# llGuy/madrona_renderer

Hardware: AMD Instinct MI355X
Metric: rendered views/sec (whole node), N worlds x 64x64 RGB+depth (higher is better)
Workload: dtype f32

## Files before the change

include/mrx.h:

```cpp
#ifndef MRX_H
#define MRX_H

#include <stddef.h>
#include <stdint.h>

#ifdef __cplusplus
extern "C" {
#endif

#define MRX_ABI_VERSION 4

enum {
    MRX_OK = 0,
    MRX_E_INVALID = -1,
    MRX_E_NO_DEVICE = -2,
    MRX_E_HIP = -3,
    MRX_E_ASSET = -4,
    MRX_E_UNSUPPORTED = -5
};

enum { MRX_MODE_RASTERIZER = 0, MRX_MODE_RAYTRACER = 1 };

typedef struct {
    float position[3];
// ... 220 lines not shown
                  uint32_t pass_rows, float *out_flow);

int mrx_copy_to_host(mrx_renderer *r, int which, void *dst, uint64_t bytes);

int mrx_refresh_objects(mrx_renderer *r);

int mrx_num_shards(mrx_renderer *r);
mrx_renderer *mrx_shard(mrx_renderer *r, int shard);
void *mrx_buffer_shard(mrx_renderer *r, int shard, int which, int64_t dims[4], int *ndim,
                       int *dtype, int *device);
int64_t mrx_shard_first_world(mrx_renderer *r, int shard);
int64_t mrx_shard_split(uint32_t num_worlds, uint32_t shard, uint32_t num_shards);

enum {
    MRX_ENTRY_NONE = 0, MRX_ENTRY_GROUP_FAST = 1, MRX_ENTRY_GROUP = 2, MRX_ENTRY_CHUNKED = 3,
    MRX_ENTRY_BRUTE = 4, MRX_ENTRY_BVH = 5
};
int mrx_raster_entry(mrx_renderer *r);
enum {
    MRX_FORM_UNIFORM = 0, MRX_FORM_PV = 1, MRX_FORM_PVL = 2, MRX_FORM_C = 3, MRX_FORM_PVLC = 4, MRX_FORM_M = 5,
    MRX_FORM_PVLM = 6, MRX_FORM_N = 7, MRX_FORM_NPV = 8, MRX_FORM_L = 9, MRX_FORM_LN = 10, MRX_FORM_PVM = 11
};
typedef struct {
    int32_t form;
    int32_t slots;
} mrx_kernel_form_t;
int mrx_kernel_form(mrx_renderer *r, mrx_kernel_form_t *out);
enum { MRX_BVH_KERNEL_NONE = 0, MRX_BVH_KERNEL_TILE = 1, MRX_BVH_KERNEL_FLAT = 2 };
typedef struct {
    int32_t kernel;
    uint32_t tile_w, tile_h;
// ... 33 lines not shown
int mrx_obj_objects(const char *path, uint32_t *first_tri, uint32_t capacity);
int mrx_decode_png(const char *path, uint8_t **rgba, uint32_t *width,
                   uint32_t *height);
int mrx_decode_texture(const char *path, uint8_t **rgba, uint32_t *width,
                       uint32_t *height);
int mrx_decode_bc7(const uint8_t *blocks, uint32_t num_blocks, uint8_t *rgba );
int64_t mrx_describe_obj_materials(const char *path, char *json, uint64_t capacity);
int mrx_blas_check(const float *tri_pos , uint32_t num_tris, uint32_t *num_nodes,
                   uint32_t *depth, uint32_t *num_leaves);
void mrx_free(void *p);
uint32_t mrx_dispatch_min_tris(uint32_t base, uint32_t num_views, int textured, uint32_t width, uint32_t height,
                               uint32_t num_cus);
uint32_t mrx_group_fill(uint32_t num_cus);
int mrx_dispatch_flat(int raytracer, uint32_t num_views, uint32_t width, uint32_t height, uint32_t max_world_triangles,
                      uint32_t max_world_instances, uint32_t num_cus);

int mrx_set_view_projection(mrx_renderer *r, uint32_t first_view, uint32_t count, const mrx_projection *proj);
int mrx_view_projection(mrx_renderer *r, uint32_t first_view, uint32_t count, mrx_projection *out);
int mrx_projection_constants(uint32_t width, uint32_t height, int render_mode, mrx_projection proj, float out[6]);

int mrx_set_world_light(mrx_renderer *r, uint32_t first_world, uint32_t count, const mrx_light *lights);
int mrx_world_light(mrx_renderer *r, uint32_t first_world, uint32_t count, mrx_light *out);
int mrx_light_constants(mrx_light light, float out[5]);

int mrx_set_instance_materials(mrx_renderer *r, uint32_t first_row, uint32_t count, const int32_t *materials);
int mrx_instance_materials(mrx_renderer *r, uint32_t first_row, uint32_t count, int32_t *out);

int mrx_set_instance_labels(mrx_renderer *r, uint32_t first_row, uint32_t count, const int32_t *labels);
int mrx_instance_labels(mrx_renderer *r, uint32_t first_row, uint32_t count, int32_t *out);

// ... 9 lines not shown
```

madrona_renderer_amd/build.py:

```python
import os
import shutil
import subprocess
import sys
import sysconfig

HERE = os.path.dirname(os.path.abspath(__file__))
ROOT = os.path.dirname(HERE)
CSRC = os.path.join(HERE, "csrc")
ARCH = "gfx950"

HIP_SOURCES = ["raster.hip", "bvh.hip", "resolve.hip", "unproject.hip", "boxes.hip", "observe.hip", "rays.hip", "rays_host.cpp", "flow.hip", "flow_host.cpp", "bvh.cpp", "mrx_api.cpp", "scene.cpp", "stages.cpp", "shards.cpp", "host_tools.cpp", "assets.cpp", "ktx2.cpp"]
HIP_DEPS = HIP_SOURCES + ["raster.hpp", "raster_dev.hpp", "bvh.hpp", "resolve.hpp", "unproject.hpp", "boxes.hpp", "observe.hpp", "rays.hpp", "rays_core.hpp", "flow.hpp", "flow_core.hpp", "assets.hpp", "bc7_tables.inc",
                          "renderer.hpp", "shards.hpp", "error.hpp",
                          "../../include/mrx.h"]
MGR_SOURCES = ["manager.cpp"]
MGR_DEPS = MGR_SOURCES + ["../../include/madrona_mi355/manager.hpp",
                          "../../include/madrona_mi355/types.hpp", "../../include/mrx.h"]
PY_SOURCES = ["py_module.cpp", "manager.cpp"]


def ext_suffix():
    return sysconfig.get_config_var("EXT_SUFFIX") or ".so"


def lib_path():
    return os.path.join(HERE, "libmrx_hip.so")

# ... 188 lines not shown
```

madrona_renderer_amd/csrc/host_tools.cpp:

```cpp
#include "renderer.hpp"

#include "assets.hpp"
#include "boxes.hpp"
#include "rays.hpp"

extern "C" {

int mrx_projection_constants(uint32_t width, uint32_t height, int render_mode, mrx_projection proj, float out[6])
{
    if (!out)
        return fail(MRX_E_INVALID, "null output");
    if (render_mode != MRX_MODE_RASTERIZER && render_mode != MRX_MODE_RAYTRACER)
        return fail(MRX_E_INVALID, "bad render_mode");
    const bool rt = render_mode == MRX_MODE_RAYTRACER;
    mrx::ViewProj c;
    const int rc = projectionConstants(width, rt ? width : height, rt, proj, c);
    if (rc != MRX_OK)
        return rc;
    out[0] = c.sx; out[1] = c.ox; out[2] = c.sz; out[3] = c.oz; out[4] = c.invNear; out[5] = c.s6bPad;
    return MRX_OK;
}

int mrx_light_constants(mrx_light light, float out[5])
{
// ... 178 lines not shown
}

uint32_t mrx_dispatch_min_tris(uint32_t base, uint32_t num_views, int textured, uint32_t width, uint32_t height,
                               uint32_t num_cus)
{
    return mrx::bvhDispatchMinTris(base ? base : mrx::kBvhMinTris, num_views, textured != 0, width, height, num_cus);
}

uint32_t mrx_group_fill(uint32_t num_cus) { return mrx::groupFill(num_cus); }

int mrx_dispatch_flat(int raytracer, uint32_t num_views, uint32_t width, uint32_t height, uint32_t max_world_triangles,
                      uint32_t max_world_instances, uint32_t num_cus)
{
    return mrx::bvhDispatchFlat(raytracer != 0, num_views, width, raytracer ? width : height, max_world_triangles,
                                max_world_instances, num_cus) ? 1 : 0;
}

int mrx_blas_check(const float *tri_pos, uint32_t num_tris, uint32_t *num_nodes, uint32_t *depth,
                   uint32_t *num_leaves)
{
    if ((!tri_pos && num_tris) || !num_nodes || !depth || !num_leaves)
        return fail(MRX_E_INVALID, "null argument");
    using namespace mrx;
    std::vector<ObjTri> tris(num_tris);
    for (uint32_t t = 0; t < num_tris; ++t)
        std::memcpy(tris[t].p, tri_pos + 9 * (size_t)t, 36);
    BlasSet b;
    buildBlas(tris.data(), { 0 }, { (int32_t)num_tris }, b);
    *num_nodes = (uint32_t)b.nodes.size();
    *depth = b.maxDepth;
// ... 66 lines not shown
```

madrona_renderer_amd/csrc/manager.cpp:

```cpp
#include "../../include/madrona_mi355/manager.hpp"
#include "../../include/mrx.h"

#include <algorithm>
#include <cstdio>
#include <cstdlib>
#include <stdexcept>
#include <string>
#include <vector>

namespace madRender {

namespace detail {
static bool g_throwOnError = false;
void setThrowOnError(bool v) { g_throwOnError = v; }

[[noreturn]] static void fatal(const char *msg)
{
    if (g_throwOnError)
        throw std::runtime_error(msg);
    std::fprintf(stderr, "FATAL: %s\n", msg);
    std::fflush(stderr);
    std::abort();
}
[[noreturn]] static void fatal(const std::string &msg) { fatal(msg.c_str()); }
// ... 302 lines not shown
    return accepted(mrx_set_instance_labels(impl_->r, first, count, labels));
}

void Manager::instanceLabels(uint32_t first, uint32_t count, int32_t *out) const
{
    check(mrx_instance_labels(impl_->r, first, count, out));
}

int Manager::placement(float *candUs, int capacity, float *keptUs) const
{
    return mrx_placement(impl_->r, candUs, capacity, keptUs);
}

const char *Manager::rasterEntry() const
{
    static const char *const names[] = {"none", "group-fast", "group", "chunked", "brute", "bvh"};
    const int e = mrx_raster_entry(impl_->r);
    if (e < 0 || e >= (int)(sizeof names / sizeof names[0]))
        detail::fatal(mrx_last_error());
    return names[e];
}

Manager::KernelFormInfo Manager::kernelForm() const
{
    static const char *const names[] = {"Uniform", "PV", "PVL", "C", "PVLC", "M", "PVLM", "N", "NPV", "L", "LN", "PVM"};
    mrx_kernel_form_t f {};
    check(mrx_kernel_form(impl_->r, &f));
    if (f.form < 0 || f.form >= (int)(sizeof names / sizeof names[0]))
        detail::fatal("mrx_kernel_form: unknown form");
    return KernelFormInfo { names[f.form], f.slots };
}
// ... 13 lines not shown
```

madrona_renderer_amd/csrc/mrx_api.cpp:

```cpp
#include "renderer.hpp"

#include <chrono>
#include <utility>

#include "boxes.hpp"
#include "observe.hpp"

constexpr size_t kOutPeriod = 512u << 10;
static size_t outPhase(const char *env, size_t dflt)
{
    if (const char *dbg = std::getenv(env))
        return (size_t)std::atoll(dbg) << 10;
    return dflt;
}
bool firstKindIsOneBlock(size_t px)
{
    if (const char *dbg = std::getenv("MRX_OUT_KIND"))
        return dbg[0] == 'o';
    return px * 4 < (128ull << 20);
}

hipError_t allocOutputs(size_t px, bool wantRgb, bool wantDepth, bool wantIds, bool oneAllocation,
                        DevBuf<uint32_t> &rgb, DevBuf<float> &depth, DevBuf<int32_t> &ids,
                        bool wantNormal, DevBuf<uint32_t> &normal)
// ... 775 lines not shown
        if (const int src = settle(r))
            return src;
    if (!r)
        return fail(MRX_E_INVALID, "null renderer");
    if (!r->shards.empty())
        return shardsRun(r, kCmdSync);
    MRX_HIP(hipSetDevice(r->device));
    MRX_HIP(hipStreamSynchronize(r->stream));
    return MRX_OK;
}

void *mrx_stream(mrx_renderer *r) { return r ? (void *)r->stream : nullptr; }

static_assert(mrx::kEntryNone == MRX_ENTRY_NONE && mrx::kEntryGroupFast == MRX_ENTRY_GROUP_FAST &&
                  mrx::kEntryGroup == MRX_ENTRY_GROUP && mrx::kEntryChunked == MRX_ENTRY_CHUNKED &&
                  mrx::kEntryBrute == MRX_ENTRY_BRUTE && mrx::kEntryBvh == MRX_ENTRY_BVH,
              "raster.hpp RasterEntry and mrx.h MRX_ENTRY_* disagree");

int mrx_raster_entry(mrx_renderer *r)
{
    if (!r)
        return fail(MRX_E_INVALID, "null renderer");
    return r->shards.empty() ? r->lastEntry : r->shards[0]->lastEntry;
}

#define MRX_FORM_SAME(name, NAME) ((int)mrx::KernelForm::name == MRX_FORM_##NAME)
static_assert(MRX_FORM_SAME(Uniform, UNIFORM) && MRX_FORM_SAME(PV, PV) && MRX_FORM_SAME(PVL, PVL) && MRX_FORM_SAME(C, C) &&
                  MRX_FORM_SAME(PVLC, PVLC) && MRX_FORM_SAME(M, M) && MRX_FORM_SAME(PVLM, PVLM) && MRX_FORM_SAME(N, N) &&
                  MRX_FORM_SAME(NPV, NPV) && MRX_FORM_SAME(L, L) && MRX_FORM_SAME(LN, LN) && MRX_FORM_SAME(PVM, PVM),
              "raster.hpp KernelForm and mrx.h MRX_FORM_* disagree");
#undef MRX_FORM_SAME
// ... 473 lines not shown
```

madrona_renderer_amd/csrc/raster.hip:

```cpp
#include <hip/hip_runtime.h>
#include <algorithm>
#include <cstdlib>

#include "raster.hpp"
#include "raster_dev.hpp"

namespace mrx {
namespace {

constexpr int kWavesPerBlock = 4;
constexpr int kBruteThreads = kWave * kWavesPerBlock;
constexpr int kChunkedThreads = kWave * kWavesPerBlock, kChunkedWavesPerSimd = 3;
constexpr int kChunk = 64;
constexpr int kHot = 16;
constexpr int kBandRows = 16;
constexpr int kBlocksPerBand = 16;

struct WaveLds {
    float hot[kChunk][kHot];
    float cold[kChunk][kCold];
};

struct TileCtx {
    uint32_t view, tileX0, tileY0;
    uint32_t triBegin, numTris;
    int lx, ly;
};

// ... 244 lines not shown
void rasterBruteKernel(const RasterParams p)
{
    bruteKernelBody<IDS, MULTI, OUT, false>(p);
}

template <KernelForm F, bool IDS, bool MULTI>
__global__ __launch_bounds__(kBruteThreads)
void rasterBruteFormKernel(const RasterParams p)
{
    static_assert(F == KernelForm::PV || F == KernelForm::N || F == KernelForm::NPV, "the forms of this family");
    bruteKernelBody<IDS, MULTI, kOutByPointer, formFlags(F).pv, formFlags(F).nrm>(p);
}

constexpr uint32_t kNearFree = 1u << 16;

template <int S0, int S1>
__device__ __forceinline__ uint32_t classifyStrips(const TriPlanes &c, uint32_t tileX0,
                                                   uint32_t tileY0, float invNear, float invFar,
                                                   bool &nearOk)
{
    const float X0 = (float)tileX0, Y0 = (float)tileY0;
    const float xa0 = c.A0 < 0.0f ? X0 : X0 + 31.0f;
    const float xa1 = c.A1 < 0.0f ? X0 : X0 + 31.0f;
    const float xa2 = c.A2 < 0.0f ? X0 : X0 + 31.0f;
    const float xdh = c.Dx < 0.0f ? X0 : X0 + 31.0f;
    const float xdl = c.Dx < 0.0f ? X0 + 31.0f : X0;
    const float yb0 = c.B0 < 0.0f ? Y0 : Y0 + 7.0f;
    const float yb1 = c.B1 < 0.0f ? Y0 : Y0 + 7.0f;
    const float yb2 = c.B2 < 0.0f ? Y0 : Y0 + 7.0f;
    const float ydh = c.Dy < 0.0f ? Y0 : Y0 + 7.0f;
    const float ydl = c.Dy < 0.0f ? Y0 + 7.0f : Y0;
    uint32_t mask = 0;
    float dmax = -__builtin_inff();
#pragma unroll
    for (int s = S0; s < S1; ++s) {
        const float dy = (float)(8 * s);
        const float r0 = __builtin_fmaf(c.B0, yb0 + dy, c.C0);
        const float r1 = __builtin_fmaf(c.B1, yb1 + dy, c.C1);
        const float r2 = __builtin_fmaf(c.B2, yb2 + dy, c.C2);
        const float rh = __builtin_fmaf(c.Dy, ydh + dy, c.Dc);
        const float rl = __builtin_fmaf(c.Dy, ydl + dy, c.Dc);
        const bool yin = (Y0 + dy + 7.0f >= c.bbY0) && (Y0 + dy <= c.bbY1);
#pragma unroll
        for (int hf = 0; hf < 2; ++hf) {
            const float dx = (float)(32 * hf);
            const float e0 = __builtin_fmaf(c.A0, xa0 + dx, r0);
            const float e1 = __builtin_fmaf(c.A1, xa1 + dx, r1);
            const float e2 = __builtin_fmaf(c.A2, xa2 + dx, r2);
            const float dh = __builtin_fmaf(c.Dx, xdh + dx, rh);
            const float dl = __builtin_fmaf(c.Dx, xdl + dx, rl);
            const bool xin = (X0 + dx + 31.0f >= c.bbX0) && (X0 + dx <= c.bbX1);
            const bool possible = (fminf(fminf(e0, e1), e2) >= 0.0f) &&
                                  (dh > invFar) && (dl <= invNear) && xin && yin;
            mask |= possible ? (1u << (2 * s + hf)) : 0u;
            dmax = fmaxf(dmax, dh);
        }
    }
    nearOk = dmax <= invNear;
    return mask;
}

__device__ __forceinline__ uint32_t classifyRegions(const TriPlanes &c, const TileCtx &t,
                                                    float invNear, float invFar)
{
    bool nearOk;
    uint32_t mask = classifyStrips<0, 8>(c, t.tileX0, t.tileY0, invNear, invFar, nearOk);
    if (nearOk)
        mask |= kNearFree;
    return mask;
}


template <bool NEAR>
__device__ __forceinline__ void pixelTest(const PlanePairs &q, f32x2 r01, f32x2 r2d, float px,
                                          float invNear, int32_t kv, float &best, int32_t &bid)
{
    const f32x2 pp = { px, px };
    const f32x2 e01 = fma2(q.A01, pp, r01);
    const f32x2 e2d = fma2(q.A2D, pp, r2d);
    bool in = (fminf(fminf(e01.x, e01.y), e2d.x) >= 0.0f) & (e2d.y > best);
    if (NEAR)
        in = in & (e2d.y <= invNear);
    best = in ? e2d.y : best;
    bid = in ? kv : bid;
}

template <bool NEAR, int IDSHIFT>
__device__ __forceinline__ void rasterRegion(const float (*planes)[16], uint64_t act, int recBase,
                                             const float (&px)[kRegionBlocks], float py,
                                             float invNear,
                                             float (&best)[kRegionBlocks],
                                             int32_t (&bid)[kRegionBlocks])
{
    const f32x2 yy = { py, py };
    for (; act != 0; act &= act - 1) {
        const int k = recBase + __builtin_ctzll(act);
        const PlanePairs q = loadPlanes(planes, k);
        const f32x2 r01 = fma2(q.B01, yy, q.C01);
        const f32x2 r2d = fma2(q.B2D, yy, q.C2D);
#pragma unroll
        for (int b = 0; b < kRegionBlocks; ++b)
            pixelTest<NEAR>(q, r01, r2d, px[b], invNear, k << IDSHIFT, best[b], bid[b]);
    }
}

template <bool IDS, bool NRM = false>
__device__ __forceinline__ void outputRegion(const RasterParams &p, const TileCtx &t,
                                             uint32_t fx0, uint32_t fy, float invFar,
                                             const float (&best)[kRegionBlocks],
                                             const uint32_t (&rgba)[kRegionBlocks],
                                             const int32_t (&id)[kRegionBlocks],
                                             const uint32_t *nrm = nullptr)
{
    float dep[kRegionBlocks];
#pragma unroll
    for (int b = 0; b < kRegionBlocks; ++b)
        dep[b] = best[b] > invFar ? __builtin_amdgcn_rcpf(best[b]) : 0.0f;
    if (fy >= p.nslow || (p.debugSkip & 1u))
        return;
// ... 175 lines not shown
    static constexpr int kRecs = SLOTS <= kChunk ? kChunk + 16 : SLOTS;
    static constexpr int kBackground = kRecs;
    float planes[kRecs][16];
    uint32_t live[kRecs];
    float shade[kRecs + 1][4];
    float cold[kRecs][kCold];
    uint32_t masks[groupTilesMax(SLOTS) * (SLOTS <= kChunk ? kChunk : SLOTS)];
    uint32_t tileInfo[kGroupTilesMax][4];
    float tileNear[PV ? kGroupTilesMax : 1];
    uint32_t nextItem;
    uint8_t itemOrder[kGroupTilesMax * 8];
    uint2 items[SLOTS == 16 ? kGroupTilesMax * 8 : 1];
    uint8_t itemPos[SLOTS == 16 ? kGroupTilesMax * 8 : 1];
};
constexpr uint32_t kTileValid = 4u;
constexpr uint32_t kItemValid = 1u << 8;
constexpr uint32_t kItemNearFree = 1u << 9;
constexpr uint32_t kItemAnyTex = 1u << 10;


template <bool IDS, bool FULL, bool TEX, int OUT, bool NRM = false, typename LDS>
__device__ __forceinline__ void storeRegion(const RasterParams &p, const LDS &L, bool doRgb, bool doDepth,
                                            uint32_t *rgbTile, float *depthTile, int32_t *idsTile,
                                            uint32_t pixOff, uint32_t fx0, uint32_t fy,
                                            bool anyTex, const float (&px)[kRegionBlocks], float py,
                                            const float (&best)[kRegionBlocks],
                                            const int32_t (&bid)[kRegionBlocks],
                                            const uint32_t *nrmTab = nullptr, uint32_t *nrmTile = nullptr)
{
    uint32_t nrm[kRegionBlocks];
    if (NRM) {
#pragma unroll
        for (int b = 0; b < kRegionBlocks; ++b)
// ... 103 lines not shown
    c.B0 = b.x; c.B1 = b.y; c.B2 = b.z; c.Dy = b.w;
    c.C0 = cc.x; c.C1 = cc.y; c.C2 = cc.z; c.Dc = cc.w;
    c.bbX0 = bb.x; c.bbX1 = bb.y; c.bbY0 = bb.z; c.bbY1 = bb.w;
    const uint32_t tx0 = L.tileInfo[j][1], ty0 = L.tileInfo[j][2];
    uint32_t m;
    switch (wave & 3) {
    case 0: m = classifyStrips<0, 2>(c, tx0, ty0, invNear, invFar, nearOk); break;
    case 1: m = classifyStrips<2, 4>(c, tx0, ty0, invNear, invFar, nearOk); break;
    case 2: m = classifyStrips<4, 6>(c, tx0, ty0, invNear, invFar, nearOk); break;
    default: m = classifyStrips<6, 8>(c, tx0, ty0, invNear, invFar, nearOk); break;
    }
    tex = __float_as_int(L.shade[rec][1]) >= 0;
    return m;
}

constexpr int groupWaves(bool tex) { return tex ? 4 : 8; }

template <bool IDS, int SLOTS, bool TEX, int XMODE, bool FAST, int OUT, bool PV = false, bool LT = false, bool COL = false,
          bool MAT = false, bool NRM = false, bool LAB = false>
__device__ __forceinline__ void groupKernelBody(const char *hPose, const char *hGeom, uint32_t hViews, uint32_t hInstances,
                                                uint32_t hPool, uint32_t hShape, uint32_t hGroups, uint32_t hPrefix,
                                                uint32_t hFirst01, uint32_t hFirst23, const RasterParams p)
{
    __shared__ GroupLds<SLOTS, PV> lds;
    constexpr int kBackground = GroupLds<SLOTS, PV>::kBackground;
    __shared__ uint32_t nrmLds[NRM ? GroupLds<SLOTS, PV>::kRecs + 1 : 1];
    const int wave = __builtin_amdgcn_readfirstlane(threadIdx.x / kWave);
    const int lane = threadIdx.x % kWave;
    if (!FAST || wave >= 2)
        touchKernelArguments<(FAST ? 48 : 0) + sizeof(RasterParams)>();
    const uint32_t aNumViews = FAST ? hViews : p.numViews;
// ... 560 lines not shown
        const dim3 grid(numGroups);
        const dim3 gblock(kWave * groupWaves(p.anyTextured != 0));
        GroupHeader h {};
        h.pose = p.poseBlock;
        h.geom = p.geomBlock;
        h.views = p.numViews;
        h.instances = p.numInstances;
        h.poolTris = p.poolTris;
        h.groups = numGroups;
        bool fast = slots == 16 && tpv == 1 && gpv == 1 && p.uniInstances != 0 && p.uniCamsPerWorld < 256 && vg < 256 &&
                    p.poseBlock && p.geomBlock && p.debugSkip == 0 && p.debugStamps == nullptr && p.uniPrefix[4] < 256;
        for (int i = 0; i < 4 && fast; ++i)
            fast = p.uniFirstTri[i] < 65536u;
        if (const char *dbg = std::getenv("MRX_GROUP_FAST"))
            fast = fast && std::atoi(dbg) != 0;
        if (entry) *entry = fast ? kEntryGroupFast : kEntryGroup;
        if (fast) {
            h.shape = vg | (q.xcdSkew << 8) | (q.xcdRotate << 12) | (p.uniInstances << 13) | (p.uniCamsPerWorld << 16) | (1u << 31);
            h.prefix = p.uniPrefix[1] | (p.uniPrefix[2] << 8) | (p.uniPrefix[3] << 16) | (p.uniPrefix[4] << 24);
            h.first01 = p.uniFirstTri[0] | (p.uniFirstTri[1] << 16);
            h.first23 = p.uniFirstTri[2] | (p.uniFirstTri[3] << 16);
        }
        const KernelForm form = groupForm(p);
        if (took) *took = LaunchForm { (int32_t)form, slots };
        const bool tex = p.anyTextured != 0;
        const OutSel out = outSelOf(p.rgb, p.depth);
        const int xmode = slots != 16 ? 0 : ((q.xcdSkew && (p.xcdPhase & 1u)) ? 1 : 0) | (p.xccReport ? 2 : 0);
        const auto byTexIds = [&](auto f) {
            withBool(tex, [&](auto TEX) { withBool(ids, [&](auto IDS) { f(IDS, TEX); }); });
        };
        const auto launchFast = [&](auto kernel) {
            kernel<<<grid, gblock, 0, stream>>>(h.pose, h.geom, h.views, h.instances, h.poolTris, h.shape, h.groups, h.prefix,
                                                h.first01, h.first23, q);
        };
        const auto launchPlain = [&](auto kernel) { kernel<<<grid, gblock, 0, stream>>>(q); };
        withValue<int, 16, 32, 64, 128, 256>(slots, [&](auto S) {
            constexpr int kSlots = decltype(S)::value;
            if (form != KernelForm::Uniform) {
                withValue<KernelForm, KernelForm::PV, KernelForm::PVL, KernelForm::C, KernelForm::PVLC, KernelForm::M,
                          KernelForm::PVLM, KernelForm::N, KernelForm::NPV, KernelForm::L, KernelForm::LN>(form, [&](auto F) {
                    constexpr KernelForm kForm = decltype(F)::value;
                    byTexIds([&](auto IDS, auto TEX) {
                        constexpr bool kIds = decltype(IDS)::value, kTex = decltype(TEX)::value;
                        if constexpr (kIds || !formFlags(kForm).lab) {
                            if constexpr (kSlots == 16) {
                                if (fast)
                                    return launchFast(rasterGroupFormKernelFast<kForm, kIds, kTex>);
                            }
                            launchPlain(rasterGroupFormKernel<kForm, kIds, kSlots, kTex>);
                        }
// ... 27 lines not shown
```

madrona_renderer_amd/csrc/raster.hpp:

```cpp
#pragma once

#include <cstdint>
#include <type_traits>
#include <hip/hip_runtime_api.h>

namespace mrx {

struct BvhNode;
struct ObjInfo;

struct alignas(32) ViewProj {
    float sx, ox, sz, oz;
    float invNear, s6bPad;
    float pad[2];
};
static_assert(sizeof(ViewProj) == 32, "ViewProj is one 32-byte record");

struct alignas(32) ViewLight {
    float toLight[3];
    float ambient, diffuse;
    float pad[3];
};
static_assert(sizeof(ViewLight) == 32, "ViewLight is one 32-byte record");

// ... 230 lines not shown
        return base < 91u ? base : 91u;
    return base;
}

inline bool bvhDispatchFlat(bool raytracer, uint32_t numViews, uint32_t nfast, uint32_t nslow, uint32_t maxWorldTris,
                            uint32_t maxWorldInstances, uint32_t numCUs)
{
    const uint32_t cus = numCUs ? numCUs : 256u;
    const uint64_t tpv = (uint64_t)((nfast + 63u) / 64u) * ((nslow + 63u) / 64u);
    return raytracer && maxWorldTris >= 1u && maxWorldTris <= 64u && maxWorldInstances <= 64u && tpv >= 16u &&
           (uint64_t)numViews * tpv >= 192ull * cus;
}

enum RasterEntry : int32_t {
    kEntryNone = 0, kEntryGroupFast = 1, kEntryGroup = 2, kEntryChunked = 3, kEntryBrute = 4, kEntryBvh = 5,
};
struct LaunchForm {
    int32_t form = 0;
    int32_t slots = 0;
};
hipError_t launchRaster(const RasterParams &p, uint32_t maxWorldTris,
                        int32_t variant, hipStream_t stream, int32_t *entry = nullptr, LaunchForm *took = nullptr);

hipError_t launchBvh(const RasterParams &p, hipStream_t stream, LaunchForm *took = nullptr);
constexpr uint32_t kBvhMaxWorldTris = 0x1FFFFEu;
size_t bvhLdsBytes(uint32_t passInst, bool textured, bool classify, uint32_t groupViews, uint32_t texCap);

struct BvhLaunchShape {
    int32_t flat;
    uint32_t tileW, tileH, classify, textured, recordCap, recordUsable, texCap, bigCap, passInst;
    uint32_t groupViews, mixed, priority, groupTiles, workgroups;
// ... 6 lines not shown
```

Baseline: 186.0 million.

## Add fixed 64x64 untextured uniform group raster kernel with compile-time resolution

Adds a specialized group rasterizer for the untextured, uniform-form, fast path at exactly 64x64 resolution with write-through output and up to four views per group. The kernel hardcodes strip and view byte strides, sizes its LDS for 16 slots per view, and writes output with inline-assembly 16-byte streaming stores using immediate offsets. Shared device helpers move into a common header. The aim is to cut address arithmetic, generic slot dispatch, and LDS footprint on the common benchmark shape. In exchange it adds another kernel variant to maintain, plus hand-written assembly stores and LDS ticket atomics.

```diff
diff --git a/include/mrx.h b/include/mrx.h
--- a/include/mrx.h
+++ b/include/mrx.h
@@ -258,7 +258,8 @@
 
 enum {
     MRX_ENTRY_NONE = 0, MRX_ENTRY_GROUP_FAST = 1, MRX_ENTRY_GROUP = 2, MRX_ENTRY_CHUNKED = 3,
-    MRX_ENTRY_BRUTE = 4, MRX_ENTRY_BVH = 5
+    MRX_ENTRY_BRUTE = 4, MRX_ENTRY_BVH = 5,
+    MRX_ENTRY_GROUP_FIXED64 = 6
 };
 int mrx_raster_entry(mrx_renderer *r);
 enum {
@@ -322,6 +323,8 @@
 uint32_t mrx_group_fill(uint32_t num_cus);
 int mrx_dispatch_flat(int raytracer, uint32_t num_views, uint32_t width, uint32_t height, uint32_t max_world_triangles,
                       uint32_t max_world_instances, uint32_t num_cus);
+int mrx_dispatch_fixed64(int fast, int textured, int form, uint32_t nfast, uint32_t nslow, uint32_t write_through,
+                         uint32_t group_views);
 
 int mrx_set_view_projection(mrx_renderer *r, uint32_t first_view, uint32_t count, const mrx_projection *proj);
 int mrx_view_projection(mrx_renderer *r, uint32_t first_view, uint32_t count, mrx_projection *out);
diff --git a/madrona_renderer_amd/build.py b/madrona_renderer_amd/build.py
--- a/madrona_renderer_amd/build.py
+++ b/madrona_renderer_amd/build.py
@@ -9,8 +9,8 @@
 CSRC = os.path.join(HERE, "csrc")
 ARCH = "gfx950"
 
-HIP_SOURCES = ["raster.hip", "bvh.hip", "resolve.hip", "unproject.hip", "boxes.hip", "observe.hip", "rays.hip", "rays_host.cpp", "flow.hip", "flow_host.cpp", "bvh.cpp", "mrx_api.cpp", "scene.cpp", "stages.cpp", "shards.cpp", "host_tools.cpp", "assets.cpp", "ktx2.cpp"]
-HIP_DEPS = HIP_SOURCES + ["raster.hpp", "raster_dev.hpp", "bvh.hpp", "resolve.hpp", "unproject.hpp", "boxes.hpp", "observe.hpp", "rays.hpp", "rays_core.hpp", "flow.hpp", "flow_core.hpp", "assets.hpp", "bc7_tables.inc",
+HIP_SOURCES = ["raster.hip", "raster_fixed.hip", "bvh.hip", "resolve.hip", "unproject.hip", "boxes.hip", "observe.hip", "rays.hip", "rays_host.cpp", "flow.hip", "flow_host.cpp", "bvh.cpp", "mrx_api.cpp", "scene.cpp", "stages.cpp", "shards.cpp", "host_tools.cpp", "assets.cpp", "ktx2.cpp"]
+HIP_DEPS = HIP_SOURCES + ["raster.hpp", "raster_dev.hpp", "raster_group_dev.hpp", "bvh.hpp", "resolve.hpp", "unproject.hpp", "boxes.hpp", "observe.hpp", "rays.hpp", "rays_core.hpp", "flow.hpp", "flow_core.hpp", "assets.hpp", "bc7_tables.inc",
                           "renderer.hpp", "shards.hpp", "error.hpp",
                           "../../include/mrx.h"]
 MGR_SOURCES = ["manager.cpp"]
diff --git a/madrona_renderer_amd/csrc/host_tools.cpp b/madrona_renderer_amd/csrc/host_tools.cpp
--- a/madrona_renderer_amd/csrc/host_tools.cpp
+++ b/madrona_renderer_amd/csrc/host_tools.cpp
@@ -216,6 +216,12 @@
 {
     return mrx::bvhDispatchFlat(raytracer != 0, num_views, width, raytracer ? width : height, max_world_triangles,
                                 max_world_instances, num_cus) ? 1 : 0;
+}
+
+int mrx_dispatch_fixed64(int fast, int textured, int form, uint32_t nfast, uint32_t nslow, uint32_t write_through,
+                         uint32_t group_views)
+{
+    return mrx::groupFixed64(fast != 0, textured != 0, (mrx::KernelForm)form, nfast, nslow, write_through, group_views) ? 1 : 0;
 }
 
 int mrx_blas_check(const float *tri_pos, uint32_t num_tris, uint32_t *num_nodes, uint32_t *depth,
diff --git a/madrona_renderer_amd/csrc/manager.cpp b/madrona_renderer_amd/csrc/manager.cpp
--- a/madrona_renderer_amd/csrc/manager.cpp
+++ b/madrona_renderer_amd/csrc/manager.cpp
@@ -340,7 +340,7 @@
 
 const char *Manager::rasterEntry() const
 {
-    static const char *const names[] = {"none", "group-fast", "group", "chunked", "brute", "bvh"};
+    static const char *const names[] = {"none", "group-fast", "group", "chunked", "brute", "bvh", "group-fast"};
     const int e = mrx_raster_entry(impl_->r);
     if (e < 0 || e >= (int)(sizeof names / sizeof names[0]))
         detail::fatal(mrx_last_error());
diff --git a/madrona_renderer_amd/csrc/mrx_api.cpp b/madrona_renderer_amd/csrc/mrx_api.cpp
--- a/madrona_renderer_amd/csrc/mrx_api.cpp
+++ b/madrona_renderer_amd/csrc/mrx_api.cpp
@@ -813,7 +813,8 @@
 
 static_assert(mrx::kEntryNone == MRX_ENTRY_NONE && mrx::kEntryGroupFast == MRX_ENTRY_GROUP_FAST &&
                   mrx::kEntryGroup == MRX_ENTRY_GROUP && mrx::kEntryChunked == MRX_ENTRY_CHUNKED &&
-                  mrx::kEntryBrute == MRX_ENTRY_BRUTE && mrx::kEntryBvh == MRX_ENTRY_BVH,
+                  mrx::kEntryBrute == MRX_ENTRY_BRUTE && mrx::kEntryBvh == MRX_ENTRY_BVH &&
+                  mrx::kEntryGroupFixed64 == MRX_ENTRY_GROUP_FIXED64,
               "raster.hpp RasterEntry and mrx.h MRX_ENTRY_* disagree");
 
 int mrx_raster_entry(mrx_renderer *r)
diff --git a/madrona_renderer_amd/csrc/raster.hip b/madrona_renderer_amd/csrc/raster.hip
--- a/madrona_renderer_amd/csrc/raster.hip
+++ b/madrona_renderer_amd/csrc/raster.hip
@@ -4,6 +4,7 @@
 
 #include "raster.hpp"
 #include "raster_dev.hpp"
+#include "raster_group_dev.hpp"
 
 namespace mrx {
 namespace {
@@ -11,7 +12,6 @@
 constexpr int kWavesPerBlock = 4;
 constexpr int kBruteThreads = kWave * kWavesPerBlock;
 constexpr int kChunkedThreads = kWave * kWavesPerBlock, kChunkedWavesPerSimd = 3;
-constexpr int kChunk = 64;
 constexpr int kHot = 16;
 constexpr int kBandRows = 16;
 constexpr int kBlocksPerBand = 16;
@@ -286,51 +286,6 @@
 
 constexpr uint32_t kNearFree = 1u << 16;
 
-template <int S0, int S1>
-__device__ __forceinline__ uint32_t classifyStrips(const TriPlanes &c, uint32_t tileX0,
-                                                   uint32_t tileY0, float invNear, float invFar,
-                                                   bool &nearOk)
-{
-    const float X0 = (float)tileX0, Y0 = (float)tileY0;
-    const float xa0 = c.A0 < 0.0f ? X0 : X0 + 31.0f;
-    const float xa1 = c.A1 < 0.0f ? X0 : X0 + 31.0f;
-    const float xa2 = c.A2 < 0.0f ? X0 : X0 + 31.0f;
-    const float xdh = c.Dx < 0.0f ? X0 : X0 + 31.0f;
-    const float xdl = c.Dx < 0.0f ? X0 + 31.0f : X0;
-    const float yb0 = c.B0 < 0.0f ? Y0 : Y0 + 7.0f;
-    const float yb1 = c.B1 < 0.0f ? Y0 : Y0 + 7.0f;
-    const float yb2 = c.B2 < 0.0f ? Y0 : Y0 + 7.0f;
-    const float ydh = c.Dy < 0.0f ? Y0 : Y0 + 7.0f;
-    const float ydl = c.Dy < 0.0f ? Y0 + 7.0f : Y0;
-    uint32_t mask = 0;
-    float dmax = -__builtin_inff();
-#pragma unroll
-    for (int s = S0; s < S1; ++s) {
-        const float dy = (float)(8 * s);
-        const float r0 = __builtin_fmaf(c.B0, yb0 + dy, c.C0);
-        const float r1 = __builtin_fmaf(c.B1, yb1 + dy, c.C1);
-        const float r2 = __builtin_fmaf(c.B2, yb2 + dy, c.C2);
-        const float rh = __builtin_fmaf(c.Dy, ydh + dy, c.Dc);
-        const float rl = __builtin_fmaf(c.Dy, ydl + dy, c.Dc);
-        const bool yin = (Y0 + dy + 7.0f >= c.bbY0) && (Y0 + dy <= c.bbY1);
-#pragma unroll
-        for (int hf = 0; hf < 2; ++hf) {
-            const float dx = (float)(32 * hf);
-            const float e0 = __builtin_fmaf(c.A0, xa0 + dx, r0);
-            const float e1 = __builtin_fmaf(c.A1, xa1 + dx, r1);
-            const float e2 = __builtin_fmaf(c.A2, xa2 + dx, r2);
-            const float dh = __builtin_fmaf(c.Dx, xdh + dx, rh);
-            const float dl = __builtin_fmaf(c.Dx, xdl + dx, rl);
-            const bool xin = (X0 + dx + 31.0f >= c.bbX0) && (X0 + dx <= c.bbX1);
-            const bool possible = (fminf(fminf(e0, e1), e2) >= 0.0f) &&
-                                  (dh > invFar) && (dl <= invNear) && xin && yin;
-            mask |= possible ? (1u << (2 * s + hf)) : 0u;
-            dmax = fmaxf(dmax, dh);
-        }
-    }
-    nearOk = dmax <= invNear;
-    return mask;
-}
 
 __device__ __forceinline__ uint32_t classifyRegions(const TriPlanes &c, const TileCtx &t,
                                                     float invNear, float invFar)
@@ -343,38 +298,6 @@
 }
 
 
-template <bool NEAR>
-__device__ __forceinline__ void pixelTest(const PlanePairs &q, f32x2 r01, f32x2 r2d, float px,
-                                          float invNear, int32_t kv, float &best, int32_t &bid)
-{
-    const f32x2 pp = { px, px };
-    const f32x2 e01 = fma2(q.A01, pp, r01);
-    const f32x2 e2d = fma2(q.A2D, pp, r2d);
-    bool in = (fminf(fminf(e01.x, e01.y), e2d.x) >= 0.0f) & (e2d.y > best);
-    if (NEAR)
-        in = in & (e2d.y <= invNear);
-    best = in ? e2d.y : best;
-    bid = in ? kv : bid;
-}
-
-template <bool NEAR, int IDSHIFT>
-__device__ __forceinline__ void rasterRegion(const float (*planes)[16], uint64_t act, int recBase,
-                                             const float (&px)[kRegionBlocks], float py,
-                                             float invNear,
-                                             float (&best)[kRegionBlocks],
-                                             int32_t (&bid)[kRegionBlocks])
-{
-    const f32x2 yy = { py, py };
-    for (; act != 0; act &= act - 1) {
-        const int k = recBase + __builtin_ctzll(act);
-        const PlanePairs q = loadPlanes(planes, k);
-        const f32x2 r01 = fma2(q.B01, yy, q.C01);
-        const f32x2 r2d = fma2(q.B2D, yy, q.C2D);
-#pragma unroll
-        for (int b = 0; b < kRegionBlocks; ++b)
-            pixelTest<NEAR>(q, r01, r2d, px[b], invNear, k << IDSHIFT, best[b], bid[b]);
-    }
-}
 
 template <bool IDS, bool NRM = false>
 __device__ __forceinline__ void outputRegion(const RasterParams &p, const TileCtx &t,
@@ -580,9 +503,6 @@
     uint8_t itemPos[SLOTS == 16 ? kGroupTilesMax * 8 : 1];
 };
 constexpr uint32_t kTileValid = 4u;
-constexpr uint32_t kItemValid = 1u << 8;
-constexpr uint32_t kItemNearFree = 1u << 9;
-constexpr uint32_t kItemAnyTex = 1u << 10;
 
 
 template <bool IDS, bool FULL, bool TEX, int OUT, bool NRM = false, typename LDS>
@@ -716,7 +636,6 @@
     return m;
 }
 
-constexpr int groupWaves(bool tex) { return tex ? 4 : 8; }
 
 template <bool IDS, int SLOTS, bool TEX, int XMODE, bool FAST, int OUT, bool PV = false, bool LT = false, bool COL = false,
           bool MAT = false, bool NRM = false, bool LAB = false>
@@ -1307,14 +1226,17 @@
             fast = p.uniFirstTri[i] < 65536u;
         if (const char *dbg = std::getenv("MRX_GROUP_FAST"))
             fast = fast && std::atoi(dbg) != 0;
-        if (entry) *entry = fast ? kEntryGroupFast : kEntryGroup;
+        const KernelForm form = groupForm(p);
+        bool fixed64 = groupFixed64(fast, p.anyTextured != 0, form, p.nfast, p.nslow, p.writeThrough, vg);
+        if (const char *dbg = std::getenv("MRX_GROUP_FIXED64"))
+            fixed64 = fixed64 && std::atoi(dbg) != 0;
+        if (entry) *entry = fixed64 ? kEntryGroupFixed64 : fast ? kEntryGroupFast : kEntryGroup;
         if (fast) {
             h.shape = vg | (q.xcdSkew << 8) | (q.xcdRotate << 12) | (p.uniInstances << 13) | (p.uniCamsPerWorld << 16) | (1u << 31);
             h.prefix = p.uniPrefix[1] | (p.uniPrefix[2] << 8) | (p.uniPrefix[3] << 16) | (p.uniPrefix[4] << 24);
             h.first01 = p.uniFirstTri[0] | (p.uniFirstTri[1] << 16);
             h.first23 = p.uniFirstTri[2] | (p.uniFirstTri[3] << 16);
         }
-        const KernelForm form = groupForm(p);
         if (took) *took = LaunchForm { (int32_t)form, slots };
         const bool tex = p.anyTextured != 0;
         const OutSel out = outSelOf(p.rgb, p.depth);
@@ -1327,6 +1249,10 @@
                                                 h.first01, h.first23, q);
         };
         const auto launchPlain = [&](auto kernel) { kernel<<<grid, gblock, 0, stream>>>(q); };
+        if (fixed64) {
+            launchRasterFixed64(h, q, numGroups, ids, xmode, out, stream);
+            return hipGetLastError();
+        }
         withValue<int, 16, 32, 64, 128, 256>(slots, [&](auto S) {
             constexpr int kSlots = decltype(S)::value;
             if (form != KernelForm::Uniform) {
diff --git a/madrona_renderer_amd/csrc/raster.hpp b/madrona_renderer_amd/csrc/raster.hpp
--- a/madrona_renderer_amd/csrc/raster.hpp
+++ b/madrona_renderer_amd/csrc/raster.hpp
@@ -268,7 +268,17 @@
 
 enum RasterEntry : int32_t {
     kEntryNone = 0, kEntryGroupFast = 1, kEntryGroup = 2, kEntryChunked = 3, kEntryBrute = 4, kEntryBvh = 5,
-};
+    kEntryGroupFixed64 = 6,
+};
+
+inline bool groupFixed64(bool fast, bool textured, KernelForm form, uint32_t nfast, uint32_t nslow, uint32_t writeThrough,
+                         uint32_t grpViews)
+{
+    return fast && !textured && form == KernelForm::Uniform && nfast == 64u && nslow == 64u && writeThrough == 1u &&
+           grpViews >= 1u && grpViews <= 4u;
+}
+void launchRasterFixed64(const GroupHeader &h, const RasterParams &q, uint32_t numGroups, bool ids, int xmode, OutSel out,
+                         hipStream_t stream);
 struct LaunchForm {
     int32_t form = 0;
     int32_t slots = 0;
diff --git a/madrona_renderer_amd/csrc/raster_fixed.hip b/madrona_renderer_amd/csrc/raster_fixed.hip
--- /dev/null
+++ b/madrona_renderer_amd/csrc/raster_fixed.hip
@@ -0,0 +1,342 @@
+#include <hip/hip_runtime.h>
+
+#include "raster.hpp"
+#include "raster_dev.hpp"
+#include "raster_group_dev.hpp"
+
+namespace mrx {
+namespace {
+
+constexpr int kFixedRes = 64;
+constexpr int kFixedSlots = 16;
+constexpr int kFixedViewsMax = 5;
+constexpr int kFixedWaves = groupWaves(false);
+constexpr uint32_t kFixedViewBytes = kFixedRes * kFixedRes * 4u;
+constexpr uint32_t kFixedStripBytes = kFixedRes * 8u * 4u;
+constexpr uint32_t kFixedHalfBytes = 32u * 4u;
+
+struct FixedLds {
+    static constexpr int kRecs = kFixedViewsMax * kFixedSlots;
+    static constexpr int kBackground = kRecs;
+    float planes[kRecs][16];
+    uint32_t live[kRecs];
+    float shade[kRecs + 1][4];
+    float cold[kRecs][kCold];
+    uint32_t nextItem;
+    uint2 items[kFixedViewsMax * 8];
+    uint8_t itemPos[kFixedViewsMax * 8];
+};
+
+struct FixedSetupArgs {
+    const ObjTri *tris;
+    const TriMat *triMats;
+    const float *instPos, *instRot, *instScale;
+    float sx, ox, sz, oz, s6bPad, ambient, diffuse;
+    int32_t transposed;
+};
+
+template <int IMM>
+__device__ __forceinline__ void streamStore16Base(const void *base, uint32_t off, uint32_t a, uint32_t b, uint32_t c,
+                                                  uint32_t d)
+{
+    const u32x4 v = { a, b, c, d };
+    asm volatile("global_store_dwordx4 %0, %1, %2 offset:%3 sc1\n\ts_nop 1" :: "v"(off), "v"(v), "s"(base), "n"(IMM) : "memory");
+}
+
+__device__ __forceinline__ uint32_t takeTicket(uint32_t *counter, int lane)
+{
+    uint32_t item = 0;
+    if (lane == 0)
+        asm volatile("ds_add_rtn_u32 %0, %1, %2\n\ts_waitcnt lgkmcnt(0)"
+                     : "=&v"(item) : "v"((uint32_t)(uintptr_t)(__attribute__((address_space(3))) uint32_t *)counter), "v"(1u)
+                     : "memory");
+    return __builtin_amdgcn_readfirstlane(item);
+}
+
+template <bool IDS, int XMODE, int OUT>
+__device__ __forceinline__ void fixedKernelBody(const char *hPose, const char *hGeom, uint32_t hViews, uint32_t hInstances,
+                                                uint32_t hPool, uint32_t hShape, uint32_t hGroups, uint32_t hPrefix,
+                                                uint32_t hFirst01, uint32_t hFirst23, const RasterParams p)
+{
+    __shared__ FixedLds lds;
+    constexpr int kBackground = FixedLds::kBackground;
+    const int wave = __builtin_amdgcn_readfirstlane(threadIdx.x / kWave);
+    const int lane = threadIdx.x % kWave;
+    if (wave >= 2)
+        touchKernelArguments<48 + sizeof(RasterParams)>();
+    const uint32_t aGrpViews = hShape & 255u;
+    const uint32_t aXcdSkew = (hShape >> 8) & 15u;
+    const uint32_t aXcdRotate = (hShape >> 12) & 1u;
+    const uint32_t aUniInstances = (hShape >> 13) & 7u;
+    const uint32_t aUniCams = (hShape >> 16) & 255u;
+    const PoseLayout lay = poseLayout(hViews, hInstances);
+    const float *aCamRot = reinterpret_cast<const float *>(hPose + lay.camRot);
+    const float *aCamPos = reinterpret_cast<const float *>(hPose + lay.camPos);
+    const int32_t *aInstObj = reinterpret_cast<const int32_t *>(hPose + lay.instObj);
+    const uint32_t blk = ((XMODE & 1) != 0 && aXcdSkew && (blockIdx.x ^ 1u) < hGroups) ? blockIdx.x ^ 1u : blockIdx.x;
+    if ((XMODE & 2) && blockIdx.x == 0 && threadIdx.x == (kFixedWaves - 1) * kWave && p.xccReport)
+        *p.xccReport = __builtin_amdgcn_s_getreg((3 << 11) | 20);
+    uint32_t bid = blk;
+    if (aXcdRotate && (bid | 7u) < hGroups)
+        bid = (bid & ~7u) | ((bid + 2u * (bid >> 3)) & 7u);
+    const uint32_t firstView = bid * aGrpViews;
+    uint32_t groupViews = aGrpViews, firstStrip = 0, numStrips = aGrpViews * 8u;
+    if (aXcdSkew) {
+        if (blk & 1u) {
+            firstStrip = aXcdSkew;
+            numStrips -= aXcdSkew;
+        } else {
+            groupViews += 1;
+            numStrips += aXcdSkew;
+        }
+    }
+    const int groupRecs = (int)groupViews * kFixedSlots;
+    const float invNear = p.invNear, invFar = p.invFar;
+
+    if (wave == kFixedWaves - 1) {
+        const uint32_t m16 = groupViews == 1 ? 65536u : groupViews == 2 ? 32768u : groupViews == 3 ? 21846u
+                             : groupViews == 4 ? 16384u : 13108u;
+        const uint32_t c = (uint32_t)lane;
+        const uint32_t strip = (c * m16) >> 16, vi = c - strip * groupViews;
+        const uint32_t g = vi * 8u + strip;
+        const bool ok = strip < 8u && g >= firstStrip && g < firstStrip + numStrips;
+        const uint64_t m = __ballot(ok);
+        const uint32_t pos = __builtin_popcountll(m & ((1ull << lane) - 1ull));
+        if (strip < 8u)
+            lds.itemPos[g] = ok ? (uint8_t)pos : (uint8_t)0xFF;
+    }
+    if (wave * kWave < groupRecs) {
+        const int rec = wave * kWave + lane;
+        const int vi = rec / kFixedSlots, k = rec % kFixedSlots;
+        const bool recOk = rec < groupRecs;
+        const bool viewOk = recOk && firstView + vi < hViews;
+        const uint32_t view = viewOk ? firstView + vi : 0u;
+        WorldTri wt;
+        uint32_t numTris;
+        {
+            const uint32_t kk = (uint32_t)k;
+            const uint32_t pre1 = hPrefix & 255u, pre2 = (hPrefix >> 8) & 255u;
+            const uint32_t pre3 = (hPrefix >> 16) & 255u, pre4 = hPrefix >> 24;
+            const uint32_t ft0 = hFirst01 & 0xFFFFu, ft1 = hFirst01 >> 16;
+            const uint32_t ft2 = hFirst23 & 0xFFFFu, ft3 = hFirst23 >> 16;
+            const uint32_t li = (kk >= pre1 ? 1u : 0u) + (kk >= pre2 ? 1u : 0u) + (kk >= pre3 ? 1u : 0u);
+            const uint32_t pre = li == 0 ? 0u : li == 1 ? pre1 : li == 2 ? pre2 : pre3;
+            const uint32_t first = li == 0 ? ft0 : li == 1 ? ft1 : li == 2 ? ft2 : ft3;
+            uint32_t world = view;
+            if (aUniCams != 1)
+                world = view / aUniCams;
+            wt.inst = world * aUniInstances + li;
+            wt.tri = first + (kk - pre);
+            numTris = viewOk ? pre4 : 0u;
+            if (kk >= pre4) {
+                wt.inst = 0;
+                wt.tri = 0;
+            }
+        }
+        ViewConst vc;
+        const ViewLight lt = viewLightOf(p, false, view);
+        {
+            const float4 q = *reinterpret_cast<const float4 *>(aCamRot + 4 * view);
+            quatToMat(q.x, q.y, q.z, q.w, vc.Rc);
+#pragma unroll
+            for (int r = 0; r < 3; ++r) {
+                vc.c[r] = aCamPos[3 * view + r];
+                vc.lv[r] = dot3(vc.Rc[0][r], vc.Rc[1][r], vc.Rc[2][r],
+                                lt.toLight[0], lt.toLight[1], lt.toLight[2]);
+            }
+        }
+        TriPlanes c;
+        c.A0 = c.B0 = c.C0 = c.A1 = c.B1 = c.C1 = 0.0f;
+        c.A2 = c.B2 = c.C2 = c.Dx = c.Dy = c.Dc = 0.0f;
+        c.bbX0 = c.bbX1 = c.bbY0 = c.bbY1 = 0.0f;
+        bool valid = false;
+        if (recOk) {
+            if ((uint32_t)k < numTris) {
+                const ViewProj pr = viewProjOf(p, false, view);
+                const FixedSetupArgs sa = {
+                    reinterpret_cast<const ObjTri *>(hGeom),
+                    reinterpret_cast<const TriMat *>(hGeom + geomMatsOffset(hPool)),
+                    reinterpret_cast<const float *>(hPose + lay.instPos),
+                    reinterpret_cast<const float *>(hPose + lay.instRot),
+                    reinterpret_cast<const float *>(hPose + lay.instScale),
+                    pr.sx, pr.ox, pr.sz, pr.oz, pr.s6bPad, lt.ambient, lt.diffuse, p.transposed };
+                InstXform x;
+                instanceTransform(sa, vc, wt.inst, x);
+                valid = setupTriangleCore<true, OUT != kOutDepth, false, false>(sa, vc.lv, x, wt.tri, aInstObj[wt.inst], k, c,
+                                                                                lds.shade[rec], lds.cold[rec]);
+            }
+            float4 *dst = reinterpret_cast<float4 *>(lds.planes[rec]);
+            dst[0] = make_float4(c.A0, c.A1, c.A2, c.Dx);
+            dst[1] = make_float4(c.B0, c.B1, c.B2, c.Dy);
+            dst[2] = make_float4(c.C0, c.C1, c.C2, c.Dc);
+            dst[3] = make_float4(c.bbX0, c.bbX1, c.bbY0, c.bbY1);
+            lds.live[rec] = valid ? 1u : 0u;
+        }
+        if (rec == 0) {
+            lds.nextItem = 0;
+            lds.shade[kBackground][0] = __uint_as_float(0xFF000000u);
+            lds.shade[kBackground][1] = __int_as_float(-1);
+            lds.shade[kBackground][2] = __int_as_float(-1);
+            lds.shade[kBackground][3] = __int_as_float(-1);
+        }
+    }
+    __syncthreads();
+
+    if ((wave >> 2) * kWave < groupRecs) {
+        const int pair = (wave >> 2) * kWave + lane;
+        const uint32_t j = (uint32_t)pair / kFixedSlots;
+        uint32_t m = 0;
+        bool nearOk = false;
+        if (pair < groupRecs && firstView + j < hViews && lds.live[pair]) {
+            const float4 *src = reinterpret_cast<const float4 *>(lds.planes[pair]);
+            const float4 a = src[0], b = src[1], cc = src[2], bb = src[3];
+            TriPlanes c;
+            c.A0 = a.x; c.A1 = a.y; c.A2 = a.z; c.Dx = a.w;
+            c.B0 = b.x; c.B1 = b.y; c.B2 = b.z; c.Dy = b.w;
+            c.C0 = cc.x; c.C1 = cc.y; c.C2 = cc.z; c.Dc = cc.w;
+            c.bbX0 = bb.x; c.bbX1 = bb.y; c.bbY0 = bb.z; c.bbY1 = bb.w;
+            switch (wave & 3) {
+            case 0: m = classifyStrips<0, 2>(c, 0u, 0u, invNear, invFar, nearOk); break;
+            case 1: m = classifyStrips<2, 4>(c, 0u, 0u, invNear, invFar, nearOk); break;
+            case 2: m = classifyStrips<4, 6>(c, 0u, 0u, invNear, invFar, nearOk); break;
+            default: m = classifyStrips<6, 8>(c, 0u, 0u, invNear, invFar, nearOk); break;
+            }
+        }
+        m >>= 4 * (wave & 3);
+        const uint64_t l0 = __ballot(m & 1u), r0 = __ballot(m & 2u), l1 = __ballot(m & 4u), r1 = __ballot(m & 8u);
+        const uint64_t near0 = __ballot((m & 3u) && !nearOk), near1 = __ballot((m & 12u) && !nearOk);
+        if (lane % kFixedSlots == 0 && pair < groupRecs) {
+            const uint32_t valid = firstView + j < hViews ? kItemValid : 0u;
+            const auto put = [&](uint32_t strip, uint64_t l, uint64_t r, uint64_t nearHit) {
+                const uint32_t pos = lds.itemPos[j * 8u + strip];
+                if (pos == 0xFFu)
+                    return;
+                const uint32_t desc = j | strip << 4 | valid | (((nearHit >> lane) & 0xFFFFu) == 0 ? kItemNearFree : 0u);
+                lds.items[pos] = make_uint2((uint32_t)((l >> lane) & 0xFFFFu) | (uint32_t)((r >> lane) & 0xFFFFu) << 16, desc);
+            };
+            put(2u * (wave & 3), l0, r0, near0);
+            put(2u * (wave & 3) + 1u, l1, r1, near1);
+        }
+    }
+    __syncthreads();
+
+    const int lx = lane & 7, ly = lane >> 3;
+    const uint32_t laneOff = ((uint32_t)ly * kFixedRes + 4u * lx) * 4u;
+    float pxTile[2][kRegionBlocks];
+#pragma unroll
+    for (int hf = 0; hf < 2; ++hf)
+#pragma unroll
+        for (int b = 0; b < kRegionBlocks; ++b)
+            pxTile[hf][b] = (float)(hf * 32 + 4 * lx + b);
+    constexpr bool doRgb = OUT != kOutDepth, doDepth = OUT != kOutRGB;
+    const char *const shadeBase = reinterpret_cast<const char *>(&lds.shade[0][0]);
+    for (;;) {
+        const uint32_t item = takeTicket(&lds.nextItem, lane);
+        if (item >= numStrips)
+            break;
+        const uint2 d = lds.items[item];
+        const uint32_t itemMasks = __builtin_amdgcn_readfirstlane(d.x);
+        const uint32_t desc = __builtin_amdgcn_readfirstlane(d.y);
+        if (!(desc & kItemValid))
+            continue;
+        const uint32_t j = desc & 15u, strip = (desc >> 4) & 7u;
+        const int recBase = (int)j * kFixedSlots;
+        const uint64_t stripOff = (uint64_t)(firstView + j) * kFixedViewBytes + strip * kFixedStripBytes;
+        const char *const rgbStrip = reinterpret_cast<const char *>(p.rgb) + stripOff;
+        const char *const depthStrip = reinterpret_cast<const char *>(p.depth) + stripOff;
+        const char *const idsStrip = reinterpret_cast<const char *>(p.ids) + stripOff;
+        const float py = (float)(strip * 8u + (uint32_t)ly);
+#pragma unroll
+        for (int hf = 0; hf < 2; ++hf) {
+            constexpr uint32_t bg = 0xFF000000u;
+            const uint64_t act = (uint64_t)((itemMasks >> (16 * hf)) & 0xFFFFu);
+            if (act == 0) {
+                if (hf == 0) {
+                    if (doRgb)
+                        streamStore16Base<0>(rgbStrip, laneOff, bg, bg, bg, bg);
+                    if (doDepth)
+                        streamStore16Base<0>(depthStrip, laneOff, 0u, 0u, 0u, 0u);
+                    if (IDS)
+                        streamStore16Base<0>(idsStrip, laneOff, ~0u, ~0u, ~0u, ~0u);
+                } else {
+                    if (doRgb)
+                        streamStore16Base<kFixedHalfBytes>(rgbStrip, laneOff, bg, bg, bg, bg);
+                    if (doDepth)
+                        streamStore16Base<kFixedHalfBytes>(depthStrip, laneOff, 0u, 0u, 0u, 0u);
+                    if (IDS)
+                        streamStore16Base<kFixedHalfBytes>(idsStrip, laneOff, ~0u, ~0u, ~0u, ~0u);
+                }
+                continue;
+            }
+            float best[kRegionBlocks];
+            int32_t bidx[kRegionBlocks];
+#pragma unroll
+            for (int b = 0; b < kRegionBlocks; ++b) {
+                best[b] = invFar;
+                bidx[b] = kBackground * 16;
+            }
+            if (desc & kItemNearFree)
+                rasterRegion<false, 4>(lds.planes, act, recBase, pxTile[hf], py, invNear, best, bidx);
+            else
+                rasterRegion<true, 4>(lds.planes, act, recBase, pxTile[hf], py, invNear, best, bidx);
+            uint32_t rgba[kRegionBlocks];
+            int32_t id[kRegionBlocks];
+            float dep[kRegionBlocks];
+#pragma unroll
+            for (int b = 0; b < kRegionBlocks; ++b) {
+                const float *h = reinterpret_cast<const float *>(shadeBase + bidx[b]);
+                if (doRgb)
+                    rgba[b] = __float_as_uint(h[0]);
+                if (IDS)
+                    id[b] = __float_as_int(p.idsAreSegmask ? h[2] : h[3]);
+                if (doDepth)
+                    dep[b] = bidx[b] != kBackground * 16 ? __builtin_amdgcn_rcpf(best[b]) : 0.0f;
+            }
+            if (hf == 0) {
+                if (doRgb)
+                    streamStore16Base<0>(rgbStrip, laneOff, rgba[0], rgba[1], rgba[2], rgba[3]);
+                if (doDepth)
+                    streamStore16Base<0>(depthStrip, laneOff, __float_as_uint(dep[0]), __float_as_uint(dep[1]),
+                                         __float_as_uint(dep[2]), __float_as_uint(dep[3]));
+                if (IDS)
+                    streamStore16Base<0>(idsStrip, laneOff, (uint32_t)id[0], (uint32_t)id[1], (uint32_t)id[2], (uint32_t)id[3]);
+            } else {
+                if (doRgb)
+                    streamStore16Base<kFixedHalfBytes>(rgbStrip, laneOff, rgba[0], rgba[1], rgba[2], rgba[3]);
+                if (doDepth)
+                    streamStore16Base<kFixedHalfBytes>(depthStrip, laneOff, __float_as_uint(dep[0]), __float_as_uint(dep[1]),
+                                                       __float_as_uint(dep[2]), __float_as_uint(dep[3]));
+                if (IDS)
+                    streamStore16Base<kFixedHalfBytes>(idsStrip, laneOff, (uint32_t)id[0], (uint32_t)id[1], (uint32_t)id[2],
+                                                       (uint32_t)id[3]);
+            }
+        }
+    }
+}
+
+template <bool IDS, int XMODE, int OUT>
+__global__ __launch_bounds__(kWave * kFixedWaves, 8)
+void rasterGroupKernelFixed64(const char *hPose, const char *hGeom, uint32_t hViews, uint32_t hInstances, uint32_t hPool,
+                              uint32_t hShape, uint32_t hGroups, uint32_t hPrefix, uint32_t hFirst01, uint32_t hFirst23,
+                              const RasterParams p)
+{
+    fixedKernelBody<IDS, XMODE, OUT>(hPose, hGeom, hViews, hInstances, hPool, hShape, hGroups, hPrefix, hFirst01, hFirst23, p);
+}
+
+}
+
+void launchRasterFixed64(const GroupHeader &h, const RasterParams &q, uint32_t numGroups, bool ids, int xmode, OutSel out,
+                         hipStream_t stream)
+{
+    const dim3 grid(numGroups), block(kWave * kFixedWaves);
+    withValue<int, 0, 1, 2, 3>(xmode, [&](auto X) {
+        withValue<int, kOutDepth, kOutRGB, kOutRGBD>(out, [&](auto O) {
+            withBool(ids, [&](auto IDS) {
+                rasterGroupKernelFixed64<decltype(IDS)::value, decltype(X)::value, decltype(O)::value><<<grid, block, 0, stream>>>(
+                    h.pose, h.geom, h.views, h.instances, h.poolTris, h.shape, h.groups, h.prefix, h.first01, h.first23, q);
+            });
+        });
+    });
+}
+
+}
diff --git a/madrona_renderer_amd/csrc/raster_group_dev.hpp b/madrona_renderer_amd/csrc/raster_group_dev.hpp
--- /dev/null
+++ b/madrona_renderer_amd/csrc/raster_group_dev.hpp
@@ -0,0 +1,96 @@
+#pragma once
+
+#include "raster_dev.hpp"
+
+namespace mrx {
+namespace {
+
+constexpr int kChunk = 64;
+
+template <int S0, int S1>
+__device__ __forceinline__ uint32_t classifyStrips(const TriPlanes &c, uint32_t tileX0,
+                                                   uint32_t tileY0, float invNear, float invFar,
+                                                   bool &nearOk)
+{
+    const float X0 = (float)tileX0, Y0 = (float)tileY0;
+    const float xa0 = c.A0 < 0.0f ? X0 : X0 + 31.0f;
+    const float xa1 = c.A1 < 0.0f ? X0 : X0 + 31.0f;
+    const float xa2 = c.A2 < 0.0f ? X0 : X0 + 31.0f;
+    const float xdh = c.Dx < 0.0f ? X0 : X0 + 31.0f;
+    const float xdl = c.Dx < 0.0f ? X0 + 31.0f : X0;
+    const float yb0 = c.B0 < 0.0f ? Y0 : Y0 + 7.0f;
+    const float yb1 = c.B1 < 0.0f ? Y0 : Y0 + 7.0f;
+    const float yb2 = c.B2 < 0.0f ? Y0 : Y0 + 7.0f;
+    const float ydh = c.Dy < 0.0f ? Y0 : Y0 + 7.0f;
+    const float ydl = c.Dy < 0.0f ? Y0 + 7.0f : Y0;
+    uint32_t mask = 0;
+    float dmax = -__builtin_inff();
+#pragma unroll
+    for (int s = S0; s < S1; ++s) {
+        const float dy = (float)(8 * s);
+        const float r0 = __builtin_fmaf(c.B0, yb0 + dy, c.C0);
+        const float r1 = __builtin_fmaf(c.B1, yb1 + dy, c.C1);
+        const float r2 = __builtin_fmaf(c.B2, yb2 + dy, c.C2);
+        const float rh = __builtin_fmaf(c.Dy, ydh + dy, c.Dc);
+        const float rl = __builtin_fmaf(c.Dy, ydl + dy, c.Dc);
+        const bool yin = (Y0 + dy + 7.0f >= c.bbY0) && (Y0 + dy <= c.bbY1);
+#pragma unroll
+        for (int hf = 0; hf < 2; ++hf) {
+            const float dx = (float)(32 * hf);
+            const float e0 = __builtin_fmaf(c.A0, xa0 + dx, r0);
+            const float e1 = __builtin_fmaf(c.A1, xa1 + dx, r1);
+            const float e2 = __builtin_fmaf(c.A2, xa2 + dx, r2);
+            const float dh = __builtin_fmaf(c.Dx, xdh + dx, rh);
+            const float dl = __builtin_fmaf(c.Dx, xdl + dx, rl);
+            const bool xin = (X0 + dx + 31.0f >= c.bbX0) && (X0 + dx <= c.bbX1);
+            const bool possible = (fminf(fminf(e0, e1), e2) >= 0.0f) &&
+                                  (dh > invFar) && (dl <= invNear) && xin && yin;
+            mask |= possible ? (1u << (2 * s + hf)) : 0u;
+            dmax = fmaxf(dmax, dh);
+        }
+    }
+    nearOk = dmax <= invNear;
+    return mask;
+}
+
+template <bool NEAR>
+__device__ __forceinline__ void pixelTest(const PlanePairs &q, f32x2 r01, f32x2 r2d, float px,
+                                          float invNear, int32_t kv, float &best, int32_t &bid)
+{
+    const f32x2 pp = { px, px };
+    const f32x2 e01 = fma2(q.A01, pp, r01);
+    const f32x2 e2d = fma2(q.A2D, pp, r2d);
+    bool in = (fminf(fminf(e01.x, e01.y), e2d.x) >= 0.0f) & (e2d.y > best);
+    if (NEAR)
+        in = in & (e2d.y <= invNear);
+    best = in ? e2d.y : best;
+    bid = in ? kv : bid;
+}
+
+template <bool NEAR, int IDSHIFT>
+__device__ __forceinline__ void rasterRegion(const float (*planes)[16], uint64_t act, int recBase,
+                                             const float (&px)[kRegionBlocks], float py,
+                                             float invNear,
+                                             float (&best)[kRegionBlocks],
+                                             int32_t (&bid)[kRegionBlocks])
+{
+    const f32x2 yy = { py, py };
+    for (; act != 0; act &= act - 1) {
+        const int k = recBase + __builtin_ctzll(act);
+        const PlanePairs q = loadPlanes(planes, k);
+        const f32x2 r01 = fma2(q.B01, yy, q.C01);
+        const f32x2 r2d = fma2(q.B2D, yy, q.C2D);
+#pragma unroll
+        for (int b = 0; b < kRegionBlocks; ++b)
+            pixelTest<NEAR>(q, r01, r2d, px[b], invNear, k << IDSHIFT, best[b], bid[b]);
+    }
+}
+
+constexpr uint32_t kItemValid = 1u << 8;
+constexpr uint32_t kItemNearFree = 1u << 9;
+constexpr uint32_t kItemAnyTex = 1u << 10;
+
+constexpr int groupWaves(bool tex) { return tex ? 4 : 8; }
+
+}
+}
```

New measurement: 191.9 million, median of 6. 1.03x the previous value.
